# James51332/OceanSimulation

Measured on AMD Instinct MI355X. Metric: height-field points/sec (N² iFFT) at 1/2/4/8 MI355X; % HBM roofline, higher is better.
Workload: dtype f32

## Files before the change

include/oceanfft.h:

```cpp
#ifndef OCEANFFT_H
#define OCEANFFT_H

#include <stddef.h>
#include <stdint.h>

#ifdef __cplusplus
extern "C" {
#endif

#define OCEAN_OK 0
#define OCEAN_ERR_INVALID 1
#define OCEAN_ERR_HIP 2
#define OCEAN_ERR_NO_DEVICE 3
#define OCEAN_ERR_OOM 4

#define OCEAN_MAX_CASCADES 64

typedef struct ocean_settings
{
  int32_t seed[2];
  float U_10;
  float theta_0;
  float F;
  float g;
// ... 44 lines not shown
int ocean_generator_set_frame_overlap(ocean_generator* gen, int enable);
int ocean_generator_frame_bytes(const ocean_generator* gen, double per_point[2]);

int ocean_generator_create_slab(ocean_generator** out, ocean_fft* fft, int rank, int ranks);
size_t ocean_generator_exchange_bytes(const ocean_generator* gen);
int ocean_generator_slab_columns(ocean_generator* gen, float timestep, int update_spectrum, float* send);
int ocean_generator_slab_rows(ocean_generator* gen, const float* recv);
int ocean_generator_slab_info(const ocean_generator* gen, int* rank, int* ranks, int* row0, int* rows);
int ocean_slab_layout(size_t texture_size, int rank, int ranks, int half, int64_t out[6]);

#define OCEAN_COMM_ID_BYTES 128
typedef struct ocean_comm ocean_comm;
int ocean_comm_unique_id(unsigned char id[OCEAN_COMM_ID_BYTES]);
int ocean_comm_create(ocean_comm** out, const unsigned char id[OCEAN_COMM_ID_BYTES], int nranks, int rank);
int ocean_comm_wrap(ocean_comm** out, void* nccl_comm, int nranks, int rank);
int ocean_comm_destroy(ocean_comm* comm);
int ocean_comm_all_to_all(ocean_comm* comm, const void* send, void* recv, size_t bytes, void* hip_stream);
int ocean_generator_slab_frame(ocean_generator* gen, ocean_comm* comm, float timestep, int update_spectrum);
int ocean_generator_slab_frame_pipelined(ocean_generator* gen, ocean_comm* comm, float timestep, int update_spectrum);
int ocean_generator_slab_flush(ocean_generator* gen);

#define OCEAN_ERR_TIMEOUT 5
#define OCEAN_PEER_HANDLE_BYTES 256
typedef struct ocean_peers ocean_peers;
int ocean_peers_create(ocean_peers** out, ocean_generator* gen);
int ocean_peers_destroy(ocean_peers* peers);
int ocean_peers_handle(const ocean_peers* peers, unsigned char handle[OCEAN_PEER_HANDLE_BYTES]);
int ocean_peers_connect(ocean_peers* peers, const unsigned char* handles);
int ocean_peers_connect_local(ocean_peers* const* all, int ranks);
int ocean_peers_set_timeout(ocean_peers* peers, int ms);
int ocean_peers_set_put_cus(ocean_peers* peers, int cus);
int ocean_peers_set_streams(ocean_peers* peers, void* column_stream, void* put_stream, void* row_stream);
int ocean_peers_set_row_cus(ocean_peers* peers, int cus);
int ocean_peers_set_put_cu_mask(ocean_peers* peers, int cus_per_xcd);
int ocean_generator_slab_frame_put(ocean_generator* gen, ocean_peers* peers, float timestep, int update_spectrum);
int ocean_generator_slab_frame_put_pipelined(ocean_generator* gen, ocean_peers* peers, float timestep,
                                             int update_spectrum);
int ocean_peers_flush(ocean_peers* peers);
int ocean_generator_slab_put_columns(ocean_generator* gen, ocean_peers* peers, float timestep, int update_spectrum);
int ocean_generator_slab_put_rows(ocean_generator* gen, ocean_peers* peers);
int ocean_peers_synchronize(ocean_peers* peers);

int ocean_peers_debug_slot(const ocean_peers* peers, int slot, void** ptr, size_t* bytes);

int ocean_frame_plan(size_t texture_size, int cascades, int32_t out[8]);

int ocean_generator_set_profiling(ocean_generator* gen, int enable);
int ocean_generator_kernel_times(ocean_generator* gen, double ms_total[3], int64_t launches[3]);
int ocean_generator_kernel_times4(ocean_generator* gen, double ms_total[4], int64_t launches[4]);

int ocean_debug_hash(const uint32_t* xy, int count, uint32_t* raw, float* uv, void* hip_stream);
int ocean_debug_copy(void* dst, const void* src, size_t bytes, int workgroups, void* hip_stream);
int ocean_debug_fft_work_limit(ocean_fft* fft, size_t bytes);

int ocean_surface_sample(ocean_generator* const* gens, const int* cascades, int count, const float* xz,
                         int64_t points, float* out);
int ocean_surface_sample_plane(ocean_generator* const* gens, const int* cascades, int count, const float camera[5],
                               int res, float* out);
int ocean_surface_query(ocean_generator* const* gens, const int* cascades, int count, const float* xz,
                        int64_t points, int iterations, float tolerance, float* out);

int ocean_generator_mip_levels(const ocean_generator* gen);
int ocean_generator_build_mips(ocean_generator* gen);
float* ocean_generator_height_mip(ocean_generator* gen, int cascade, int level);
float* ocean_generator_displacement_mip(ocean_generator* gen, int cascade, int level);
float* ocean_generator_jacobian_mip(ocean_generator* gen, int cascade, int level);
int ocean_surface_sample_lod(ocean_generator* const* gens, const int* cascades, int count, const float* xzf,
                             int64_t points, float* out);
int ocean_surface_sample_plane_lod(ocean_generator* const* gens, const int* cascades, int count,
                                   const float camera[5], int res, float* out);

int ocean_generator_calculate_rates(ocean_generator* gen);
float* ocean_generator_height_rate_map(ocean_generator* gen, int cascade);
float* ocean_generator_displacement_rate_map(ocean_generator* gen, int cascade);
int ocean_surface_velocity(ocean_generator* const* gens, const int* cascades, int count, const float* xz,
                           int64_t points, float* out);

int ocean_generator_set_depth_layers(ocean_generator* gen, const float* depths, int layers);
int ocean_generator_depth_layers(const ocean_generator* gen, float out[8]);
int ocean_generator_calculate_kinematics(ocean_generator* gen);
float* ocean_generator_kinematics_map(ocean_generator* gen, int cascade, int layer, int image);
int ocean_water_kinematics(ocean_generator* const* gens, const int* cascades, int count, const float* xyz,
                           int64_t points, int iterations, float tolerance, float* out);

int ocean_generator_build_bounds(ocean_generator* gen);
int ocean_generator_bounds(ocean_generator* gen, int cascade, float out[18]);
const float* ocean_generator_bounds_device(ocean_generator* gen);
int ocean_surface_raycast(ocean_generator* const* gens, const int* cascades, int count, const float* rays,
                          int64_t n_rays, float step, int max_steps, int refine, int iterations, float tolerance,
                          float slope, float pad, float* out);

typedef struct ocean_camera
{
  float position[3];
  float right[3], up[3], forward[3];
  float tan_half_fov_y, near_plane, far_plane;
  float lod_scale;
} ocean_camera;
typedef struct ocean_shading
{
  float wave_color[3], scatter_color[3], sky_color[3], light_color[3], light_direction[3];
  float sun_view_angle, sun_falloff_angle, fog_begin, fog_density;
} ocean_shading;
typedef struct ocean_march
{
  float step;
// ... 115 lines not shown
```

oceansimulation_amd/capi.py:

```python
from __future__ import annotations

import ctypes
import os

_HERE = os.path.dirname(os.path.abspath(__file__))
LIB_PATH = os.path.join(_HERE, "liboceanfft.so")

OCEAN_OK = 0
OCEAN_ERR_INVALID = 1
OCEAN_ERR_HIP = 2
OCEAN_ERR_NO_DEVICE = 3
OCEAN_ERR_OOM = 4
OCEAN_ERR_TIMEOUT = 5
OCEAN_MAX_CASCADES = 64
OCEAN_COMM_ID_BYTES = 128
OCEAN_PEER_HANDLE_BYTES = 256


class OceanSettings(ctypes.Structure):

    _fields_ = [
        ("seed", ctypes.c_int32 * 2),
        ("U_10", ctypes.c_float),
        ("theta_0", ctypes.c_float),
# ... 121 lines not shown
        ("foam_hi", ctypes.c_float),
        ("foam_opacity", ctypes.c_float),
        ("spray_color", ctypes.c_float * 3),
        ("spray_radius", ctypes.c_float),
        ("spray_max_half", ctypes.c_int32),
        ("spray_opacity", ctypes.c_float),
    ]


assert ctypes.sizeof(OceanCameraLayers) == 48

_vp = ctypes.c_void_p
_i = ctypes.c_int
_f = ctypes.c_float
_sz = ctypes.c_size_t
_fp = ctypes.POINTER(ctypes.c_float)
_sp = ctypes.POINTER(OceanSettings)
_fsp = ctypes.POINTER(OceanFoamSettings)

SIGNATURES = {
    "ocean_last_error": (ctypes.c_char_p, []),
    "ocean_version": (ctypes.c_char_p, []),
    "ocean_default_settings": (None, [_sp]),
    "ocean_device_count": (_i, []),
    "ocean_fft_create": (_i, [ctypes.POINTER(_vp), _sz, _vp]),
    "ocean_fft_destroy": (_i, [_vp]),
    "ocean_fft_texture_resolution": (_sz, [_vp]),
    "ocean_fft_encode_ifft": (_i, [_vp, _vp]),
    "ocean_fft_encode_ifft_batch": (_i, [_vp, _vp, _i]),
    "ocean_fft_synchronize": (_i, [_vp]),
    "ocean_fft_device_cus": (_i, [_vp]),
    "ocean_fft_set_cu_budget": (_i, [_vp, _i]),
    "ocean_generator_create": (_i, [ctypes.POINTER(_vp), _vp, _i]),
    "ocean_generator_destroy": (_i, [_vp]),
    "ocean_generator_cascades": (_i, [_vp]),
    "ocean_generator_settings": (_sp, [_vp, _i]),
    "ocean_generator_calculate": (_i, [_vp, _f, _i]),
    "ocean_generator_generate_spectrum": (_i, [_vp]),
    "ocean_generator_height_map": (_vp, [_vp, _i]),
    "ocean_generator_displacement_map": (_vp, [_vp, _i]),
    "ocean_generator_jacobian_map": (_vp, [_vp, _i]),
    "ocean_generator_initial_spectrum": (_vp, [_vp, _i]),
    "ocean_generator_spectrum_block": (_i, [_vp]),
    "ocean_generator_create_slab": (_i, [ctypes.POINTER(_vp), _vp, _i, _i]),
    "ocean_generator_exchange_bytes": (_sz, [_vp]),
    "ocean_generator_slab_columns": (_i, [_vp, _f, _i, _vp]),
    "ocean_generator_slab_rows": (_i, [_vp, _vp]),
    "ocean_generator_slab_info": (_i, [_vp, ctypes.POINTER(_i), ctypes.POINTER(_i), ctypes.POINTER(_i), ctypes.POINTER(_i)]),
    "ocean_generator_set_profiling": (_i, [_vp, _i]),
    "ocean_generator_kernel_times": (_i, [_vp, ctypes.POINTER(ctypes.c_double), ctypes.POINTER(ctypes.c_int64)]),
    "ocean_debug_hash": (_i, [_vp, _i, _vp, _vp, _vp]),
    "ocean_debug_copy": (_i, [_vp, _vp, _sz, _i, _vp]),
    "ocean_debug_fft_work_limit": (_i, [_vp, _sz]),
    "ocean_surface_sample": (_i, [_vp, _vp, _i, _vp, ctypes.c_int64, _vp]),
    "ocean_surface_sample_plane": (_i, [_vp, _vp, _i, _vp, _i, _vp]),
    "ocean_surface_query": (_i, [_vp, _vp, _i, _vp, ctypes.c_int64, _i, ctypes.c_float, _vp]),
    "ocean_generator_mip_levels": (_i, [_vp]),
    "ocean_generator_build_mips": (_i, [_vp]),
    "ocean_generator_height_mip": (_vp, [_vp, _i, _i]),
    "ocean_generator_displacement_mip": (_vp, [_vp, _i, _i]),
    "ocean_generator_jacobian_mip": (_vp, [_vp, _i, _i]),
    "ocean_surface_sample_lod": (_i, [_vp, _vp, _i, _vp, ctypes.c_int64, _vp]),
    "ocean_surface_sample_plane_lod": (_i, [_vp, _vp, _i, _vp, _i, _vp]),
    "ocean_generator_calculate_rates": (_i, [_vp]),
    "ocean_generator_height_rate_map": (_vp, [_vp, _i]),
    "ocean_generator_displacement_rate_map": (_vp, [_vp, _i]),
    "ocean_surface_velocity": (_i, [_vp, _vp, _i, _vp, ctypes.c_int64, _vp]),
    "ocean_generator_set_depth_layers": (_i, [_vp, _fp, _i]),
    "ocean_generator_depth_layers": (_i, [_vp, _fp]),
    "ocean_generator_calculate_kinematics": (_i, [_vp]),
    "ocean_generator_kinematics_map": (_vp, [_vp, _i, _i, _i]),
    "ocean_water_kinematics": (_i, [_vp, _vp, _i, _vp, ctypes.c_int64, _i, ctypes.c_float, _vp]),
    "ocean_generator_build_bounds": (_i, [_vp]),
    "ocean_generator_bounds": (_i, [_vp, _i, _fp]),
    "ocean_generator_bounds_device": (_vp, [_vp]),
    "ocean_surface_raycast": (_i, [_vp, _vp, _i, _vp, ctypes.c_int64, _f, _i, _i, _i, _f, _f, _f, _vp]),
    "ocean_default_camera": (None, [ctypes.POINTER(OceanCamera)]),
    "ocean_default_shading": (None, [ctypes.POINTER(OceanShading)]),
    "ocean_default_march": (None, [ctypes.POINTER(OceanMarch)]),
    "ocean_camera_rays": (_i, [ctypes.POINTER(OceanCamera), _i, _i, _vp, _vp]),
    "ocean_camera_render": (_i, [_vp, _vp, _i, ctypes.POINTER(OceanCamera), ctypes.POINTER(OceanShading),
                                 ctypes.POINTER(OceanMarch), _i, _i, _vp, _vp, _vp]),
    "ocean_default_camera_layers": (None, [ctypes.POINTER(OceanCameraLayers)]),
    "ocean_camera_layers_scratch_bytes": (_sz, [_i, _i]),
    "ocean_camera_render_layers": (_i, [_vp, _vp, _i, ctypes.POINTER(OceanCamera), ctypes.POINTER(OceanShading),
                                        ctypes.POINTER(OceanMarch), ctypes.POINTER(OceanCameraLayers), _i, _i, _vp, _vp,
                                        ctypes.c_int64, _vp, _vp, _vp, _vp, _vp]),
    "ocean_default_foam_settings": (None, [_fsp]),
    "ocean_generator_foam_settings": (_fsp, [_vp, _i]),
    "ocean_generator_advance_foam": (_i, [_vp, _f]),
    "ocean_generator_reset_foam": (_i, [_vp]),
    "ocean_generator_foam_map": (_vp, [_vp, _i]),
    "ocean_generator_foam_counts": (_i, [_vp, _i, ctypes.POINTER(ctypes.c_int64)]),
    "ocean_generator_foam_counts_device": (_vp, [_vp]),
    "ocean_surface_sample_foam": (_i, [_vp, _vp, _i, _vp, ctypes.c_int64, _vp]),
    "ocean_surface_sample_plane_foam": (_i, [_vp, _vp, _i, _vp, _i, _vp]),
    "ocean_default_foam_deposit_settings": (None, [ctypes.POINTER(OceanFoamDepositSettings)]),
    "ocean_foam_deposit": (_i, [_vp, _vp, _i, ctypes.POINTER(OceanFoamDepositSettings), _vp, _vp, ctypes.c_int64]),
    "ocean_foam_deposit_counts": (_i, [_vp, ctypes.POINTER(ctypes.c_int64)]),
    "ocean_foam_deposit_counts_device": (_vp, [_vp]),
    "ocean_debug_foam_deposit_merge": (_i, [_i]),
    "ocean_hulls_create":(_i, [ctypes.POINTER(_vp), _vp, _vp, ctypes.c_int64, _vp, _i]),
    "ocean_hulls_destroy": (_i, [_vp]),
    "ocean_hulls_bodies": (_i, [_vp]),
    "ocean_hulls_instance_points": (ctypes.c_int64, [_vp]),
    "ocean_debug_hulls_packing": (_i, [_i]),
# ... 82 lines not shown
```

oceansimulation_amd/csrc/device/fft.h:

```cpp
#pragma once

#include <hip/hip_runtime.h>

#include <cstdint>

#include "device/memory.h"

namespace oceanfft
{

__device__ __forceinline__ float2 operator+(float2 a, float2 b) { return make_float2(a.x + b.x, a.y + b.y); }
__device__ __forceinline__ float2 operator-(float2 a, float2 b) { return make_float2(a.x - b.x, a.y - b.y); }
__device__ __forceinline__ float4 operator+(float4 a, float4 b)
{
  return make_float4(a.x + b.x, a.y + b.y, a.z + b.z, a.w + b.w);
}
__device__ __forceinline__ float4 operator-(float4 a, float4 b)
{
  return make_float4(a.x - b.x, a.y - b.y, a.z - b.z, a.w - b.w);
}
__device__ __forceinline__ float2 mul_i(float2 a) { return make_float2(-a.y, a.x); }
__device__ __forceinline__ float4 mul_i(float4 a) { return make_float4(-a.y, a.x, -a.w, a.z); }
__device__ __forceinline__ float2 mul_mi(float2 a) { return make_float2(a.y, -a.x); }
__device__ __forceinline__ float4 mul_mi(float4 a) { return make_float4(a.y, -a.x, a.w, -a.z); }
// ... 275 lines not shown
#pragma unroll
    for (int u = 0; u < U; u++)
    {
      V w[R0];
#pragma unroll
      for (int t = 0; t < R0; t++)
        w[t] = v[u + t * U];
      if constexpr (R0 == 2)
        idft2(w[0], w[1]);
      else if constexpr (R0 == 4)
        idft4(w[0], w[1], w[2], w[3]);
      else
        idft8(w);
#pragma unroll
      for (int t = 0; t < R0; t++)
        v[u + t * U] = w[t];
    }
    exchange<LOGN, CI, SPLIT, WAVE>(v, reg, i2, reg2, lds, [&](int q) {
      int u = q % U, t = q / U;
      return pad16((i + u * T) * R0 + t);
    });
  }

  int p = R0;
#pragma unroll
  for (int s = 1; s < S::NSTAGE; s++)
  {
    const int k = i2 & (p - 1);
    const int stride = N / (16 * p);
    apply_stage_twiddles<LOGN>(v, k * stride, tw);
    idft16(v);
    if (s + 1 < S::NSTAGE)
    {
      const int j = (i2 / p) * 16 * p + k;
      const int pp = p;
      if (pp >= 16)
      {
        const int base = pad16(j), st = pp + pp / 16;
        exchange<LOGN, CI, SPLIT, WAVE>(v, reg2, i2, reg2, lds, [&](int t) { return base + t * st; });
      }
      else
        exchange<LOGN, CI, SPLIT, WAVE>(v, reg2, i2, reg2, lds, [&](int t) { return pad16(j + t * pp); });
    }
    p *= 16;
  }
}

template <int LOGN, int CI, bool SPLIT, typename V>
__device__ __forceinline__ void fft_run(V* v, int i, int reg, void* lds, const float2* __restrict__ tw)
{
  fft_run<LOGN, CI, SPLIT>(v, i, reg, i, reg, lds, tw);
}

template <int LOGN, int CI>
__device__ __forceinline__ void exchange_x2(CPair* va, CPair* vb, int reg, void* lds_raw, int ia, int ib, int base_a,
                                            int base_b, int st)
{
  using S = FftShape<LOGN>;
  float2* lds = reinterpret_cast<float2*>(lds_raw);
#pragma unroll
  for (int half = 0; half < 2; half++)
  {
#pragma unroll
    for (int t = 0; t < 16; t++)
    {
      lds[lds_slot<CI, S::PADDED>(reg, base_a + t * st)] = half_of(va[t], half);
      lds[lds_slot<CI, S::PADDED>(reg, base_b + t * st)] = half_of(vb[t], half);
    }
    XSYNC();
#pragma unroll
    for (int m = 0; m < 16; m++)
    {
      set_half(va[m], half, lds[lds_slot<CI, S::PADDED>(reg, read_pidx<LOGN>(ia, m))]);
      set_half(vb[m], half, lds[lds_slot<CI, S::PADDED>(reg, read_pidx<LOGN>(ib, m))]);
    }
    XSYNC();
  }
}

template <int LOGN, int CI>
__device__ __forceinline__ void fft_run_x2(CPair* va, CPair* vb, int ia, int reg, void* lds, const float2* __restrict__ tw)
{
  using S = FftShape<LOGN>;
  constexpr int N = S::N, T = S::T;
  static_assert(S::R0 == 16 && CI > 0, "radix-16 stages, column layout");
  const int ib = ia + T / 2;
  idft16(va);
  idft16(vb);
  exchange_x2<LOGN, CI>(va, vb, reg, lds, ia, ib, 17 * ia, 17 * ib, 1);
  int p = 16;
#pragma unroll
  for (int s = 1; s < S::NSTAGE; s++)
  {
    const int stride = N / (16 * p);
    apply_stage_twiddles<LOGN>(va, (ia & (p - 1)) * stride, tw);
    apply_stage_twiddles<LOGN>(vb, (ib & (p - 1)) * stride, tw);
    idft16(va);
    idft16(vb);
    if (s + 1 < S::NSTAGE)
    {
      const int ja = (ia / p) * 16 * p + (ia & (p - 1)), jb = (ib / p) * 16 * p + (ib & (p - 1));
      exchange_x2<LOGN, CI>(va, vb, reg, lds, ia, ib, pad16(ja), pad16(jb), p + p / 16);
    }
    p *= 16;
  }
}
// ... 12 lines not shown
```

oceansimulation_amd/csrc/device/k_half_cols.h:

```cpp
#pragma once

#include <hip/hip_runtime.h>

#include <cstdint>

#include "ocean_internal.h"
#include "launch_common.h"
#include "device/evolve.h"
#include "device/fft.h"
#include "device/grid.h"
#include "device/memory.h"
#include "device/spectrum.h"

namespace oceanfft
{


template <int LOGN>
struct HalfCfg
{
  static constexpr int N = 1 << LOGN;
  static constexpr int B = ColFirstCfg<LOGN>::B;
  static constexpr int STRIPS = N / (2 * B) + 1;
  static constexpr bool SUPPORTED = B == 4 && ColFirstCfg<LOGN>::SPW == 1;
  static constexpr bool SLAB_SUPPORTED = ColFirstCfg<LOGN>::SPW == 1;
};

constexpr int kHalfRG = 2, kHalfRGC = 4;
constexpr int kHalfRG2 = 4, kHalfRGC2 = 8;
constexpr int kHalfHL = 1, kHalfHK = 4, kHalfHKSeed = 2;
template <int LOGN, int RG, int FB = 4>
__device__ __forceinline__ int half_group_offset(int y, int strip, int b = 0)
{
  constexpr int N = HalfCfg<LOGN>::N, FS = HalfCfg<LOGN>::STRIPS * HalfCfg<LOGN>::B / FB;
  return RG == 1 ? (strip * N + y) * FB + b : (((y / RG) * FS + strip) * RG + (y % RG)) * FB + b;
}


template <int LOGN_, bool SEED_>
struct ColsWhole
{
  static constexpr int LOGN = LOGN_, LA = SEED_ ? 0 : kStream;
  static constexpr bool SLAB = false, SEED = SEED_, PUT = false, NYQ = true;
  static constexpr int RG = kHalfRG, RGC = kHalfRGC, FB = 4;
  static constexpr int CPI = ColFirstCfg<LOGN_>::B, HB = ColFirstCfg<LOGN_>::B;
  static constexpr int HL = kHalfHL, HK = SEED_ ? kHalfHKSeed : LOGN_ == 12 ? kHalfHK : 2;
};

template <int LOGN_, bool SEED_, int HB_>
struct ColsHalfStrip
{
  static constexpr int LOGN = LOGN_, LA = SEED_ ? 0 : kStream;
  static constexpr bool SLAB = false, SEED = SEED_, PUT = false, NYQ = true;
  static constexpr int RG = kHalfRG2, RGC = kHalfRGC2, FB = 2;
  static constexpr int CPI = 2, HB = HB_;
  static constexpr int HL = kHalfHL, HK = SEED_ ? kHalfHKSeed : LOGN_ == 12 ? kHalfHK : 2;
};

template <int LOGN_, bool PUT_>
struct ColsSlab
{
  static constexpr int LOGN = LOGN_, LA = kStream;
  static constexpr bool SLAB = true, SEED = false, PUT = PUT_, NYQ = false;
  static constexpr int RG = 1, RGC = 1, FB = 4;
  static constexpr int CPI = ColFirstCfg<LOGN_>::B, HB = ColFirstCfg<LOGN_>::B;
  static constexpr int HL = kHalfHL, HK = LOGN_ == 13 ? 1 : kHalfHK - 1;
};

template <typename Sh>
struct ColsLaunch
{
  using S = FftShape<Sh::LOGN>;
  static constexpr int WG = S::T * Sh::CPI;
  static constexpr int LDS = ((S::TW_ENTRIES * 8 + 15) / 16) * 16 + Sh::CPI * S::PADDED * 8 + Sh::HL * WG * 16;
  static constexpr int items(int cascades, int nstrips) { return cascades * nstrips * (ColFirstCfg<Sh::LOGN>::B / Sh::CPI); }
  static constexpr int max_grid(int hs_blocks) { return Sh::SLAB ? hs_blocks : hs_blocks * (1024 / WG); }
};

template <typename Sh>
__global__ __launch_bounds__(ColsLaunch<Sh>::WG, Sh::CPI < ColFirstCfg<Sh::LOGN>::B ? 4 : 1) void k_cols_half(
    FrameParams fp, const float4* __restrict__ h0, float4* __restrict__ gab, float4* __restrict__ gde,
    float2* __restrict__ gc, const float2* __restrict__ tw_glob, float2* __restrict__ hs, HalfSlab hsl,
    unsigned char* __restrict__ send, int h0_full, const SpectrumConsts* __restrict__ seed)
{
  constexpr int LOGN = Sh::LOGN, LA = Sh::LA, RG = Sh::RG, RGC = Sh::RGC, CPI = Sh::CPI, HL = Sh::HL, HK = Sh::HK,
                FB = Sh::FB, HB = Sh::HB;
  constexpr bool SLAB = Sh::SLAB, SEED = Sh::SEED, PUT = Sh::PUT, NYQ = Sh::NYQ;
  using S = FftShape<LOGN>;
  using K = ColFirstCfg<LOGN>;
  using HC = HalfCfg<LOGN>;
  constexpr int N = S::N, T = S::T, B = K::B, STRIPS = HC::STRIPS, WG = T * CPI, HALVES = B / CPI;
  static_assert(SLAB ? HC::SLAB_SUPPORTED : HC::SUPPORTED, "half-spectrum path: one strip per item (B = 4 unless SLAB)");
  static_assert(CPI * HALVES == B && HALVES <= 2 && (HALVES == 1 || !SLAB), "whole or half strips");
  static_assert(HL >= 0 && HK >= 0 && HL + HK <= 8, "H pairs outside the scratch");
  static_assert(FB == 4 || (FB == CPI && HALVES == 2 && !SLAB && RG > 1 && RGC > 1), "FB: half-strip fields");
  static_assert(!PUT || SLAB, "PUT: the strip-dealt slab stores");
  static_assert(HB == B || (HB == CPI && HALVES == 2 && !SLAB), "HB: half strips over 2-column h0 strips");
  static_assert(!NYQ || !SLAB, "NYQ: whole grids (send is the spec output)");
  constexpr int XB = CPI * S::PADDED * 8;
  extern __shared__ __attribute__((aligned(16))) unsigned char smem[];
  float2* tw = reinterpret_cast<float2*>(smem);
  void* xch = smem + ((S::TW_ENTRIES * 8 + 15) / 16) * 16;
  float4* hlds = reinterpret_cast<float4*>(static_cast<unsigned char*>(xch) + XB);
  load_twiddles<LOGN>(tw, tw_glob);

  const int nstrips = SLAB ? hsl.nstrips : STRIPS;
  const int total = fp.cascades * nstrips * HALVES;
  const float dim = (float)N;
  for (int item = HALVES > 1 ? xcd_pair_slot(blockIdx.x, gridDim.x) : (int)blockIdx.x; item < total; item += gridDim.x)
  {
    const int hh = HALVES > 1 ? item % HALVES : 0, si = HALVES > 1 ? item / HALVES : item;
    const int c = si / nstrips, s = si - c * nstrips;
    const int sg = SLAB ? hsl.strip0 + s : s;
    if (HALVES > 1 && sg == STRIPS - 1 && hh != 0)
      continue;
    const int b = opaque((int)threadIdx.x) % CPI + hh * CPI;
    const int xb = sg == STRIPS - 1 ? 0 : N / (2 * B) + sg;
    const CascadeFrame f = fp.c[c];
    const float4* src = HB != B                  ? h0 + ((size_t)c * (N / HB) + xb * (B / HB) + hh) * N * HB
                        : (!SLAB || h0_full) ? h0 + ((size_t)c * (N / B) + xb) * N * B
                                             : h0 + ((size_t)c * nstrips + s) * N * B;
    const int fs = FB == 4 ? s : 2 * s + hh;
    const size_t gbase = RG == 1 ? ((size_t)c * STRIPS + s) * N * B
                                 : (size_t)c * STRIPS * N * B + half_group_offset<LOGN, RG, FB>(0, fs);
    const size_t cgbase = RGC == 1 ? ((size_t)c * STRIPS + s) * N * B
                                   : (size_t)c * STRIPS * N * B + half_group_offset<LOGN, RGC, FB>(0, fs);
    const int bf = FB == 4 ? b : b - hh * CPI;
    const int x = xb * B + b;
    float4 hk[HK > 0 ? HK : 1];
    auto run_round = [&](int round) __attribute__((always_inline)) {
      const int i = (opaque((int)threadIdx.x) / CPI) % T;
      const int voff = (i * B + b) * 16;
      CPair v[16];
      auto pack = [&](int m, float2 H, const KVec& q) __attribute__((always_inline)) {
        if (round == 0)
          v[m] = CPair{f2v{H.x, q.kz * H.x}, f2v{H.y, q.kz * H.y}};
        else if (round == 1)
        {
          const float e = q.kz * q.dirz;
          v[m] = CPair{f2v{q.dirz * H.x, e * H.x}, f2v{q.dirz * H.y, e * H.y}};
        }
        else
          v[m] = CPair{f2v{q.inv * H.x, 0.0f}, f2v{q.inv * H.y, 0.0f}};
      };
      if (SEED && round == 0)
      {
        float2* hsb = hs + (size_t)blockIdx.x * 16 * WG;
        const int hoff = opaque((int)threadIdx.x) * 8;
        const SpectrumConsts q = seed[c];
#pragma unroll 1
        for (int m = 0; m < 16; m++)
        {
          const int y = i + ((m + 8) & 15) * T;
          const float2 H = evolve(seed_texel(q, x, y, dim), make_kvec(x, y, dim, f.dk).k, f);
          if ((m >> 1) < HL)
            reinterpret_cast<float2*>(hlds)[((m >> 1) * WG + threadIdx.x) * 2 + (m & 1)] = H;
          else
            st2s<0>(hsb, hoff * 2 + (m & 1) * 8, (m >> 1) * WG * 16, H);
        }
        __threadfence_block();
#pragma unroll
        for (int m = 0; m < 16; m += 2)
        {
          const int y = i + ((m + 8) & 15) * T, p = m >> 1;
          const float4 pp = p < HL ? hlds[p * WG + threadIdx.x] : ld4s<kStream>(hsb, hoff * 2, p * WG * 16);
          if (p >= HL && p < HL + HK)
            hk[p < HL + HK && p >= HL ? p - HL : 0] = pp;
          pack(m, make_float2(pp.x, pp.y), make_kvec(x, y, dim, f.dk));
          pack(m + 1, make_float2(pp.z, pp.w), make_kvec(x, y + T, dim, f.dk));
        }
      }
      else if (round == 0)
      {
        float2* hsb = hs + (size_t)blockIdx.x * 16 * WG;
        const int hoff = opaque((int)threadIdx.x) * 8;
        float4 a[16];
        float2 hprev = make_float2(0.0f, 0.0f);
        const int loff = HB == B ? voff : (i * HB + (b - hh * CPI)) * 16;
#pragma unroll
        for (int m = 0; m < 16; m++)
          a[m] = ld4s<LA>(src, loff, ((m + 8) & 15) * T * HB * 16);
#pragma unroll
        for (int m = 0; m < 16; m++)
        {
          const int y = i + ((m + 8) & 15) * T;
          const KVec q = make_kvec(x, y, dim, f.dk);
          const float2 H = evolve(a[m], q.k, f);
          const int p = m >> 1;
          if ((m & 1) && p < HL)
            hlds[p * WG + threadIdx.x] = make_float4(hprev.x, hprev.y, H.x, H.y);
          else if ((m & 1) && p < HL + HK)
            hk[p - HL] = make_float4(hprev.x, hprev.y, H.x, H.y);
          else if (m & 1)
            st4s<0>(hsb, hoff * 2, p * WG * 16, make_float4(hprev.x, hprev.y, H.x, H.y));
          else
            hprev = H;
          pack(m, H, q);
        }
      }
      else
      {
        const float2* hsb = hs + (size_t)blockIdx.x * 16 * WG;
        const int hoff = opaque((int)threadIdx.x) * 8;
#pragma unroll
        for (int m = 0; m < 16; m += 2)
        {
          const int y = i + ((m + 8) & 15) * T, pi = m >> 1;
          const float4 p = pi < HL        ? hlds[pi * WG + threadIdx.x]
                           : pi < HL + HK ? hk[pi < HL + HK ? pi - HL : 0]
                                          : ld4s<kStream>(hsb, hoff * 2, pi * WG * 16);
          pack(m, make_float2(p.x, p.y), make_kvec(x, y, dim, f.dk));
          pack(m + 1, make_float2(p.z, p.w), make_kvec(x, y + T, dim, f.dk));
        }
      }
      const int reg = HALVES > 1 ? opaque((int)threadIdx.x) % CPI : b;
      fft_run<LOGN, CPI, true>(v, i, reg, xch, tw);
      const int vo = (i * B + b) * 16;
#pragma unroll
      for (int m = 0; m < 16; m++)
      {
        if constexpr (SLAB)
        {
          const size_t part = (size_t)fp.cascades * hsl.S * hsl.w * B;
          const int q = (m * T) / hsl.w, yl0 = (m * T) % hsl.w;
          const size_t el = (((size_t)c * hsl.S + s) * hsl.w + yl0) * B;
          unsigned char* blk =
              PUT ? reinterpret_cast<unsigned char*>(sopaque((size_t)reinterpret_cast<const uint64_t*>(send)[q]))
                  : send + sopaque((size_t)q * (part * 40 + (size_t)fp.cascades * 2 * N * 16));
          if (round == 0)
            st4<kStream>(blk + el * 16, vo, pair_raw(v[m]));
          else if (round == 1)
            st4<kStream>(blk + part * 16 + el * 16, vo, pair_raw(v[m]));
          else
            st2<kStream>(blk + part * 32 + el * 8, (i * B + b) * 8, make_float2(v[m].re.x, v[m].im.x));
        }
        else if constexpr (RG == 1 && RGC == 1)
        {
          if (round == 0)
            st4s<kStream>(gab + gbase, vo, m * T * B * 16, pair_raw(v[m]));
          else if (round == 1)
            st4s<kStream>(gde + gbase, vo, m * T * B * 16, pair_raw(v[m]));
          else
            st2s<kStream>(gc + gbase, (i * B + b) * 8, m * T * B * 8, make_float2(v[m].re.x, v[m].im.x));
        }
        else if (round == 0)
          st4s<kStream>(gab + gbase, half_group_offset<LOGN, RG, FB>(i, 0, bf) * 16, half_group_offset<LOGN, RG, FB>(m * T, 0) * 16,
                        pair_raw(v[m]));
        else if (round == 1)
          st4s<kStream>(gde + gbase, half_group_offset<LOGN, RG, FB>(i, 0, bf) * 16, half_group_offset<LOGN, RG, FB>(m * T, 0) * 16,
                        pair_raw(v[m]));
        else
          st2s<kStream>(gc + cgbase, half_group_offset<LOGN, RGC, FB>(i, 0, bf) * 8, half_group_offset<LOGN, RGC, FB>(m * T, 0) * 8,
                        make_float2(v[m].re.x, v[m].im.x));
      }
    };
#pragma unroll
    for (int round = 0; round < 3; round++)
      run_round(round);
  }
  if constexpr (NYQ)
    if ((HALVES > 1 ? xcd_pair_slot(blockIdx.x, gridDim.x) : (int)blockIdx.x) == (int)gridDim.x - 1)
      for (int idx = threadIdx.x; idx < fp.cascades * N; idx += WG)
        half_nyquist_texel(fp, N, HB, h0, reinterpret_cast<float4*>(send), nullptr, 1, 0, seed, nullptr, 0, idx);
}

template <typename Sh>
hipError_t launch_cols_half(const FrameParams& fp, int nstrips, const float4* h0, float4* gab, float4* gde, float2* gc,
                            const float2* tw, float2* hs, int hs_blocks, const HalfSlab& hsl, unsigned char* send,
                            int h0_full, const SpectrumConsts* seed, hipStream_t stream, int cus)
{
  using G = ColsLaunch<Sh>;
  auto kern = k_cols_half<Sh>;
  int grid = persistent_grid(kern, G::WG, G::LDS, G::items(fp.cascades, nstrips), cus);
  if (grid > G::max_grid(hs_blocks))
    grid = G::max_grid(hs_blocks);
  if (grid < 1)
    return hipErrorInvalidValue;
  hipLaunchKernelGGL(kern, dim3(grid), dim3(G::WG), G::LDS, stream, fp, h0, gab, gde, gc, tw, hs, hsl, send, h0_full, seed);
  return hipGetLastError();
}

}
```

oceansimulation_amd/csrc/device/memory.h:

```cpp
#pragma once

#include <hip/hip_runtime.h>

#include <cstdint>


namespace oceanfft
{

typedef float f4v __attribute__((ext_vector_type(4)));

__device__ __forceinline__ __amdgpu_buffer_rsrc_t srd(const void* base, int num_bytes)
{
  return __builtin_amdgcn_make_buffer_rsrc(const_cast<void*>(base), 0, num_bytes, 0x00020000);
}

constexpr int kAllBytes = 0x7FFFFFFF;

template <int AUX = 0>
__device__ __forceinline__ float4 ld4(const void* base, int voff_bytes, int num_bytes = kAllBytes)
{
  f4v r = __builtin_amdgcn_raw_buffer_load_b128(srd(base, num_bytes), voff_bytes, 0, AUX);
  return make_float4(r.x, r.y, r.z, r.w);
}
// ... 22 lines not shown
}

template <int AUX = 0>
__device__ __forceinline__ void st1(void* base, int voff_bytes, float v)
{
  __builtin_amdgcn_raw_buffer_store_b32(__float_as_uint(v), srd(base, kAllBytes), voff_bytes, 0, AUX);
}

#if defined(OCEAN_SOFFSET_PIECES)
#define OCEAN_PIECE(voff, soff) (voff), (soff)
#else
#define OCEAN_PIECE(voff, soff) (voff) + (soff), 0
#endif
template <int AUX = 0>
__device__ __forceinline__ float4 ld4s(const void* base, int voff_bytes, int soff_bytes)
{
  f4v r = __builtin_amdgcn_raw_buffer_load_b128(srd(base, kAllBytes), OCEAN_PIECE(voff_bytes, soff_bytes), AUX);
  return make_float4(r.x, r.y, r.z, r.w);
}

template <int AUX = 0>
__device__ __forceinline__ void st4s(void* base, int voff_bytes, int soff_bytes, float4 v)
{
  f4v r = {v.x, v.y, v.z, v.w};
  __builtin_amdgcn_raw_buffer_store_b128(r, srd(base, kAllBytes), OCEAN_PIECE(voff_bytes, soff_bytes), AUX);
}

template <int AUX = 0>
__device__ __forceinline__ float2 ld2s(const void* base, int voff_bytes, int soff_bytes)
{
  u2v r = __builtin_amdgcn_raw_buffer_load_b64(srd(base, kAllBytes), OCEAN_PIECE(voff_bytes, soff_bytes), AUX);
  return make_float2(__uint_as_float(r.x), __uint_as_float(r.y));
}

template <int AUX = 0>
__device__ __forceinline__ void st2s(void* base, int voff_bytes, int soff_bytes, float2 v)
{
  u2v r = {__float_as_uint(v.x), __float_as_uint(v.y)};
  __builtin_amdgcn_raw_buffer_store_b64(r, srd(base, kAllBytes), OCEAN_PIECE(voff_bytes, soff_bytes), AUX);
}

__device__ __forceinline__ int clamp_bytes(int64_t b)
{
  return b > kAllBytes ? kAllBytes : (b < 0 ? 0 : (int)b);
}


__device__ __forceinline__ int opaque(int v)
{
  asm volatile("" : "+v"(v));
  return v;
}

__device__ __forceinline__ size_t sopaque(size_t v)
{
  asm volatile("" : "+s"(v));
  return v;
}

__device__ __forceinline__ int sopaque(int v)
{
  asm volatile("" : "+s"(v));
  return v;
}

}
```

oceansimulation_amd/csrc/launch_half.hip:

```cpp
#include <hip/hip_runtime.h>

#include <cstdint>

#include "oceanfft.h"
#include "ocean_internal.h"
#include "launch_common.h"
#include "device/grid.h"
#include "device/k_half_cols.h"
#include "device/k_half_rows.h"
#include "device/k_rows_hp.h"
#include "device/spectrum.h"

namespace oceanfft
{

bool half_spectrum_supported(int logn) { return logn >= 10 && logn <= 12; }

constexpr bool half_strip_launch(int logn, int cascades) { return (logn == 12 || logn == 11) && cascades <= 2; }

template <int LOGN, typename V>
hipError_t select_half_cols(int cascades, bool seed, int h0_blk, V&& visit)
{
  constexpr int B = ColFirstCfg<LOGN>::B;
  if constexpr (LOGN == 12 || LOGN == 11)
// ... 25 lines not shown

template <int LOGN, typename V>
hipError_t select_half_rows(int cascades, V&& visit)
{
  const bool hs = half_strip_launch(LOGN, cascades);
  if constexpr (LOGN == 12)
    return hs ? visit(RowsHp<2, kHalfRG2, kHalfRGC2, kHalfRGC2, 0, 4>{}) : visit(RowsHp<4, kHalfRG, kHalfRGC, 4, 1, 3>{});
  else if constexpr (LOGN == 11)
    return hs ? visit(RowsHalf<2, kHalfRG2, kHalfRGC2>{}) : visit(RowsHalf<4, kHalfRG, kHalfRGC>{});
  else
    return visit(RowsHalf<4, kHalfRG, kHalfRGC>{});
}

int half_h0_block(int logn, int cascades)
{
  int hb = spectrum_block(logn);
  (void)with_logn(logn, [&](auto L) -> hipError_t {
    constexpr int LOGN = decltype(L)::value;
    if constexpr (HalfCfg<LOGN>::SUPPORTED)
      return select_half_cols<LOGN>(cascades, false, 0, [&](auto sh) {
        hb = decltype(sh)::HB;
        return hipSuccess;
      });
    else
      return hipSuccess;
  });
  return hb;
}

size_t half_field_texels(int logn)
{
  const size_t n = (size_t)1 << logn;
  return (n / 8 + 1) * n * 4;
}

size_t half_hs_bytes(int logn, int blocks)
{
  return half_slab_supported(logn) ? (size_t)blocks * 16 * 1024 * sizeof(float2) : 0;
}

hipError_t launch_half_columns(int logn, const FrameParams& fp, const float4* h0, float4* gab, float4* gcd, float2* ge,
                               float4* spec, const float2* tw, hipStream_t stream, int cus, float2* hs, int hs_blocks,
                               const void* seed_consts, int h0_blk)
{
  if (!hs)
    return hipErrorInvalidValue;
  const SpectrumConsts* seed = static_cast<const SpectrumConsts*>(seed_consts);
  return with_logn(logn, [&](auto L) -> hipError_t {
    constexpr int LOGN = decltype(L)::value;
    if constexpr (!HalfCfg<LOGN>::SUPPORTED)
      return hipErrorInvalidValue;
    else
      return select_half_cols<LOGN>(fp.cascades, seed != nullptr, h0_blk > 0 ? h0_blk : ColFirstCfg<LOGN>::B, [&](auto sh) {
        return launch_cols_half<decltype(sh)>(fp, HalfCfg<LOGN>::STRIPS, h0, gab, gcd, ge, tw, hs, hs_blocks, HalfSlab{},
                                              reinterpret_cast<unsigned char*>(spec), 1, seed, stream, cus);
      });
  });
}

hipError_t launch_half_rows(int logn, const FrameParams& fp, const float4* gab, const float4* gcd, const float2* ge,
                            const float4* rcorr, float4* maps, float* jac, const FoamParams& foam, const float2* tw,
                            hipStream_t stream, int cus)
{
  return with_logn(logn, [&](auto L) -> hipError_t {
    constexpr int LOGN = decltype(L)::value;
    if constexpr (!HalfCfg<LOGN>::SUPPORTED)
      return hipErrorInvalidValue;
    else
      return select_half_rows<LOGN>(fp.cascades, [&](auto sh) {
        using R = decltype(sh);
        using S = FftShape<LOGN>;
        if constexpr (R::HP)
        {
          auto kern = k_rows_hp<R::RG, R::RGC, false, R::FB, R::GRP, R::EARLY, R::MINB>;
          const int grid = persistent_grid(kern, 256, HpCfg::LDS, fp.cascades * S::N, cus);
          hipLaunchKernelGGL(kern, dim3(grid), dim3(256), HpCfg::LDS, stream, fp, gab, gcd, ge, rcorr, maps, jac, foam, tw, 0,
                             RowSrc{});
        }
        else
        {
          auto kern = k_rows_half<LOGN, 0, false, R::RG, R::RGC, R::FB>;
          const int lds = ((S::TW_ENTRIES * 8 + 15) / 16) * 16 + lds_row_slots<LOGN>(2) * 8;
          const int grid = persistent_grid(kern, S::T * 2, lds, fp.cascades * (S::N / 2), cus);
          hipLaunchKernelGGL(kern, dim3(grid), dim3(S::T * 2), lds, stream, fp, gab, gcd, ge, rcorr, maps, jac, foam, tw, S::N,
                             RowSrc{});
        }
        return hipGetLastError();
      });
  });
}

}

extern "C" int ocean_frame_plan(size_t texture_size, int cascades, int32_t out[8])
{
  using namespace oceanfft;
  int logn = 0;
  while (logn < 15 && ((size_t)1 << logn) < texture_size)
    logn++;
  if (!out || ((size_t)1 << logn) != texture_size || !half_spectrum_supported(logn) || cascades < 1 ||
      cascades > kMaxCascades)
    return OCEAN_ERR_INVALID;
  const hipError_t e = with_logn(logn, [&](auto L) -> hipError_t {
    constexpr int LOGN = decltype(L)::value;
    if constexpr (!HalfCfg<LOGN>::SUPPORTED)
      return hipErrorInvalidValue;
    else
// ... 20 lines not shown
```

oceansimulation_amd/csrc/ocean_capi.cpp:

```cpp
#include "oceanfft.h"

#include <hip/hip_runtime.h>

#include <algorithm>
#include <cmath>
#include <cstdio>
#include <cstring>
#include <string>
#include <vector>

#include "ocean_capi_internal.h"
#include "ocean_internal.h"

static_assert(sizeof(ocean_settings) == sizeof(OceanSettings), "settings layout");

namespace
{
int log2_exact(size_t n)
{
  int l = 0;
  while (((size_t)1 << l) < n)
    l++;
  return ((size_t)1 << l) == n ? l : -1;
}
// ... 224 lines not shown
{
  if (!fft)
    return fail(OCEAN_ERR_INVALID, "ocean_fft_synchronize: null plan");
  HIP_TRY(hipStreamSynchronize(fft->stream), "hipStreamSynchronize");
  return OCEAN_OK;
}

}

namespace
{
hipEvent_t take_event(ocean_generator* g)
{
  if (!g->pool.empty())
  {
    hipEvent_t e = g->pool.back();
    g->pool.pop_back();
    return e;
  }
  hipEvent_t e = nullptr;
  (void)hipEventCreate(&e);
  return e;
}

template <typename F>
hipError_t timed(ocean_generator* g, int kind, F&& launch, hipStream_t stream = nullptr)
{
  if (!g->profiling)
    return launch();
  if (!stream)
    stream = g->fft->stream;
  EventPair p{kind, take_event(g), take_event(g)};
  hipError_t e = hipEventRecord(p.a, stream);
  if (e != hipSuccess)
    return e;
  e = launch();
  if (e != hipSuccess)
    return e;
  e = hipEventRecord(p.b, stream);
  g->pending.push_back(p);
  return e;
}

hipError_t half_fields(ocean_generator* g, int slot)
{
  const size_t t = half_field_texels(g->fft->logn) * g->cascades;
  HalfFields& f = g->fields[slot];
  hipError_t e = alloc_if_null(f.gab, t * sizeof(float4));
  e = alloc_if_null(f.gde, t * sizeof(float4), e);
  e = alloc_if_null(f.gc, t * sizeof(float2), e);
  return alloc_if_null(f.spec, (size_t)g->cascades * 2 * g->fft->n * sizeof(float4), e);
}

hipError_t half_buffers(ocean_generator* g)
{
  return alloc_if_null(g->hs, half_hs_bytes(g->fft->logn, g->fft->device_cus), half_fields(g, 0));
}

HalfSlab half_slab_geom(int logn, int rank, int ranks)
{
  const int strips = half_strips(logn);
  HalfSlab h{};
  h.S = (strips + ranks - 1) / ranks;
  h.strip0 = rank * h.S;
  h.nstrips = std::max(0, std::min(h.S, strips - h.strip0));
  h.w = (1 << logn) / ranks;
  return h;
}

int h0_block(const ocean_generator* g)
{
  switch (frame_path(g))
  {
    case FramePath::FourStep:
      return gen4_h0_block();
    case FramePath::HalfBlocked:
      return half_h0_block(g->fft->logn, g->cascades);
    default:
      return spectrum_block(g->fft->logn);
  }
}

size_t h0_texels(const ocean_generator* g)
{
  const size_t full = (size_t)g->fft->n * g->geom.w;
  if (g->ranks == 1)
    return full;
  const size_t strips = (size_t)g->hsl.nstrips * spectrum_block(g->fft->logn) * g->fft->n;
  size_t t = std::max(full, strips);
  if (gen4_supported(g->fft->logn))
    t = std::max(t, g->g4.h0_cstride);
  return t;
}

hipError_t full_buffers(ocean_generator* g)
{
  const size_t slab = (size_t)g->fft->n * g->geom.w * g->cascades;
  hipError_t e = alloc_if_null(g->inter, slab * 2 * sizeof(float4));
  return rows_need_transpose(g->fft->logn) ? alloc_if_null(g->scratch, slab * 2 * sizeof(float4), e) : e;
}

hipError_t path_buffers(ocean_generator* g)
{
  switch (frame_path(g))
  {
    case FramePath::Full:
// ... 825 lines not shown
```

Baseline: 61.37 billion.

## Carry the last column strip into spare FFT lanes of the third round for N=1024

For the 1024 whole-grid column kernel, the last strip is no longer given its own work items. Blocks with s==0 or s==1 compute that strip's extra fields in the unused .y lanes of the round-2 FFT and store them separately. The Nyquist texel pass is also spread across all blocks instead of running on the last block only. This aims to remove a tail of poorly occupied work and improve load balance, at the cost of extra registers, h0 loads, and opaque scheduling barriers in the round-2 path.

```diff
diff --git a/include/oceanfft.h b/include/oceanfft.h
--- a/include/oceanfft.h
+++ b/include/oceanfft.h
@@ -120,6 +120,7 @@
 int ocean_debug_hash(const uint32_t* xy, int count, uint32_t* raw, float* uv, void* hip_stream);
 int ocean_debug_copy(void* dst, const void* src, size_t bytes, int workgroups, void* hip_stream);
 int ocean_debug_fft_work_limit(ocean_fft* fft, size_t bytes);
+int ocean_debug_fill_half_fields(ocean_generator* gen, int byte);
 
 int ocean_surface_sample(ocean_generator* const* gens, const int* cascades, int count, const float* xz,
                          int64_t points, float* out);
diff --git a/oceansimulation_amd/capi.py b/oceansimulation_amd/capi.py
--- a/oceansimulation_amd/capi.py
+++ b/oceansimulation_amd/capi.py
@@ -197,6 +197,7 @@
     "ocean_debug_hash": (_i, [_vp, _i, _vp, _vp, _vp]),
     "ocean_debug_copy": (_i, [_vp, _vp, _sz, _i, _vp]),
     "ocean_debug_fft_work_limit": (_i, [_vp, _sz]),
+    "ocean_debug_fill_half_fields": (_i, [_vp, _i]),
     "ocean_surface_sample": (_i, [_vp, _vp, _i, _vp, ctypes.c_int64, _vp]),
     "ocean_surface_sample_plane": (_i, [_vp, _vp, _i, _vp, _i, _vp]),
     "ocean_surface_query": (_i, [_vp, _vp, _i, _vp, ctypes.c_int64, _i, ctypes.c_float, _vp]),
diff --git a/oceansimulation_amd/csrc/device/fft.h b/oceansimulation_amd/csrc/device/fft.h
--- a/oceansimulation_amd/csrc/device/fft.h
+++ b/oceansimulation_amd/csrc/device/fft.h
@@ -351,6 +351,79 @@
   fft_run<LOGN, CI, SPLIT>(v, i, reg, i, reg, lds, tw);
 }
 
+template <int LOGN, typename V>
+__device__ __forceinline__ void fft_stage0(V* v)
+{
+  using S = FftShape<LOGN>;
+  constexpr int R0 = S::R0;
+  if constexpr (R0 == 16)
+    idft16(v);
+  else
+  {
+    constexpr int U = 16 / R0;
+#pragma unroll
+    for (int u = 0; u < U; u++)
+    {
+      V w[R0];
+#pragma unroll
+      for (int t = 0; t < R0; t++)
+        w[t] = v[u + t * U];
+      if constexpr (R0 == 2)
+        idft2(w[0], w[1]);
+      else if constexpr (R0 == 4)
+        idft4(w[0], w[1], w[2], w[3]);
+      else
+        idft8(w);
+#pragma unroll
+      for (int t = 0; t < R0; t++)
+        v[u + t * U] = w[t];
+    }
+  }
+}
+
+template <int LOGN, int CI, bool SPLIT, typename V>
+__device__ __forceinline__ void fft_after_stage0(V* v, int i, int reg, void* lds, const float2* __restrict__ tw)
+{
+  using S = FftShape<LOGN>;
+  constexpr int N = S::N, T = S::T, R0 = S::R0;
+  static_assert(S::NSTAGE > 1, "a transform with an exchange");
+  if constexpr (R0 == 16)
+  {
+    const int base = 17 * i;
+    exchange<LOGN, CI, SPLIT>(v, reg, i, reg, lds, [&](int t) { return base + t; });
+  }
+  else
+  {
+    constexpr int U = 16 / R0;
+    exchange<LOGN, CI, SPLIT>(v, reg, i, reg, lds, [&](int q) {
+      int u = q % U, t = q / U;
+      return pad16((i + u * T) * R0 + t);
+    });
+  }
+  int p = R0;
+#pragma unroll
+  for (int s = 1; s < S::NSTAGE; s++)
+  {
+    const int k = i & (p - 1);
+    const int stride = N / (16 * p);
+    apply_stage_twiddles<LOGN>(v, k * stride, tw);
+    idft16(v);
+    if (s + 1 < S::NSTAGE)
+    {
+      const int j = (i / p) * 16 * p + k;
+      const int pp = p;
+      if (pp >= 16)
+      {
+        const int base = pad16(j), st = pp + pp / 16;
+        exchange<LOGN, CI, SPLIT>(v, reg, i, reg, lds, [&](int t) { return base + t * st; });
+      }
+      else
+        exchange<LOGN, CI, SPLIT>(v, reg, i, reg, lds, [&](int t) { return pad16(j + t * pp); });
+    }
+    p *= 16;
+  }
+}
+
 template <int LOGN, int CI>
 __device__ __forceinline__ void exchange_x2(CPair* va, CPair* vb, int reg, void* lds_raw, int ia, int ib, int base_a,
                                             int base_b, int st)
diff --git a/oceansimulation_amd/csrc/device/k_half_cols.h b/oceansimulation_amd/csrc/device/k_half_cols.h
--- a/oceansimulation_amd/csrc/device/k_half_cols.h
+++ b/oceansimulation_amd/csrc/device/k_half_cols.h
@@ -3,6 +3,7 @@
 #include <hip/hip_runtime.h>
 
 #include <cstdint>
+#include <type_traits>
 
 #include "ocean_internal.h"
 #include "launch_common.h"
@@ -41,7 +42,7 @@
 struct ColsWhole
 {
   static constexpr int LOGN = LOGN_, LA = SEED_ ? 0 : kStream;
-  static constexpr bool SLAB = false, SEED = SEED_, PUT = false, NYQ = true;
+  static constexpr bool SLAB = false, SEED = SEED_, PUT = false, NYQ = true, CARRY = !SEED_ && LOGN_ == 10;
   static constexpr int RG = kHalfRG, RGC = kHalfRGC, FB = 4;
   static constexpr int CPI = ColFirstCfg<LOGN_>::B, HB = ColFirstCfg<LOGN_>::B;
   static constexpr int HL = kHalfHL, HK = SEED_ ? kHalfHKSeed : LOGN_ == 12 ? kHalfHK : 2;
@@ -51,7 +52,7 @@
 struct ColsHalfStrip
 {
   static constexpr int LOGN = LOGN_, LA = SEED_ ? 0 : kStream;
-  static constexpr bool SLAB = false, SEED = SEED_, PUT = false, NYQ = true;
+  static constexpr bool SLAB = false, SEED = SEED_, PUT = false, NYQ = true, CARRY = false;
   static constexpr int RG = kHalfRG2, RGC = kHalfRGC2, FB = 2;
   static constexpr int CPI = 2, HB = HB_;
   static constexpr int HL = kHalfHL, HK = SEED_ ? kHalfHKSeed : LOGN_ == 12 ? kHalfHK : 2;
@@ -61,7 +62,7 @@
 struct ColsSlab
 {
   static constexpr int LOGN = LOGN_, LA = kStream;
-  static constexpr bool SLAB = true, SEED = false, PUT = PUT_, NYQ = false;
+  static constexpr bool SLAB = true, SEED = false, PUT = PUT_, NYQ = false, CARRY = false;
   static constexpr int RG = 1, RGC = 1, FB = 4;
   static constexpr int CPI = ColFirstCfg<LOGN_>::B, HB = ColFirstCfg<LOGN_>::B;
   static constexpr int HL = kHalfHL, HK = LOGN_ == 13 ? 1 : kHalfHK - 1;
@@ -73,19 +74,26 @@
   using S = FftShape<Sh::LOGN>;
   static constexpr int WG = S::T * Sh::CPI;
   static constexpr int LDS = ((S::TW_ENTRIES * 8 + 15) / 16) * 16 + Sh::CPI * S::PADDED * 8 + Sh::HL * WG * 16;
+  static constexpr int GRID_STRIPS = HalfCfg<Sh::LOGN>::STRIPS - (Sh::CARRY ? 1 : 0);
   static constexpr int items(int cascades, int nstrips) { return cascades * nstrips * (ColFirstCfg<Sh::LOGN>::B / Sh::CPI); }
   static constexpr int max_grid(int hs_blocks) { return Sh::SLAB ? hs_blocks : hs_blocks * (1024 / WG); }
 };
 
+__device__ __forceinline__ float quad_odd(float v)
+{
+  const int r = __float_as_int(v);
+  return __int_as_float(__builtin_amdgcn_update_dpp(r, r, 0xF5 , 0xF, 0xF, true));
+}
+
 template <typename Sh>
-__global__ __launch_bounds__(ColsLaunch<Sh>::WG, Sh::CPI < ColFirstCfg<Sh::LOGN>::B ? 4 : 1) void k_cols_half(
+__global__ __launch_bounds__(ColsLaunch<Sh>::WG, Sh::CPI < ColFirstCfg<Sh::LOGN>::B || Sh::CARRY ? 4 : 1) void k_cols_half(
     FrameParams fp, const float4* __restrict__ h0, float4* __restrict__ gab, float4* __restrict__ gde,
     float2* __restrict__ gc, const float2* __restrict__ tw_glob, float2* __restrict__ hs, HalfSlab hsl,
     unsigned char* __restrict__ send, int h0_full, const SpectrumConsts* __restrict__ seed)
 {
   constexpr int LOGN = Sh::LOGN, LA = Sh::LA, RG = Sh::RG, RGC = Sh::RGC, CPI = Sh::CPI, HL = Sh::HL, HK = Sh::HK,
                 FB = Sh::FB, HB = Sh::HB;
-  constexpr bool SLAB = Sh::SLAB, SEED = Sh::SEED, PUT = Sh::PUT, NYQ = Sh::NYQ;
+  constexpr bool SLAB = Sh::SLAB, SEED = Sh::SEED, PUT = Sh::PUT, NYQ = Sh::NYQ, CARRY = Sh::CARRY;
   using S = FftShape<LOGN>;
   using K = ColFirstCfg<LOGN>;
   using HC = HalfCfg<LOGN>;
@@ -97,6 +105,8 @@
   static_assert(!PUT || SLAB, "PUT: the strip-dealt slab stores");
   static_assert(HB == B || (HB == CPI && HALVES == 2 && !SLAB), "HB: half strips over 2-column h0 strips");
   static_assert(!NYQ || !SLAB, "NYQ: whole grids (send is the spec output)");
+  static_assert(!CARRY || (!SLAB && !SEED && HALVES == 1 && B == 4 && FB == 4 && HB == B && RG > 1 && RGC > 1),
+                "CARRY: whole strips of whole grids that load h0");
   constexpr int XB = CPI * S::PADDED * 8;
   extern __shared__ __attribute__((aligned(16))) unsigned char smem[];
   float2* tw = reinterpret_cast<float2*>(smem);
@@ -104,7 +114,7 @@
   float4* hlds = reinterpret_cast<float4*>(static_cast<unsigned char*>(xch) + XB);
   load_twiddles<LOGN>(tw, tw_glob);
 
-  const int nstrips = SLAB ? hsl.nstrips : STRIPS;
+  const int nstrips = SLAB ? hsl.nstrips : CARRY ? STRIPS - 1 : STRIPS;
   const int total = fp.cascades * nstrips * HALVES;
   const float dim = (float)N;
   for (int item = HALVES > 1 ? xcd_pair_slot(blockIdx.x, gridDim.x) : (int)blockIdx.x; item < total; item += gridDim.x)
@@ -128,7 +138,8 @@
     const int bf = FB == 4 ? b : b - hh * CPI;
     const int x = xb * B + b;
     float4 hk[HK > 0 ? HK : 1];
-    auto run_round = [&](int round) __attribute__((always_inline)) {
+    auto run_round = [&](int round, auto cy) __attribute__((always_inline)) {
+      constexpr int CY = decltype(cy)::value;
       const int i = (opaque((int)threadIdx.x) / CPI) % T;
       const int voff = (i * B + b) * 16;
       CPair v[16];
@@ -214,7 +225,56 @@
         }
       }
       const int reg = HALVES > 1 ? opaque((int)threadIdx.x) % CPI : b;
-      fft_run<LOGN, CPI, true>(v, i, reg, xch, tw);
+      if constexpr (CY != 0)
+      {
+        fft_stage0<LOGN>(v);
+#pragma unroll
+        for (int m = 0; m < 16; m++)
+          v[m].re.x = fopaque(v[m].re.x), v[m].im.x = fopaque(v[m].im.x);
+        CPair w[16];
+        const int cf = CY == 2 ? 4 : b;
+        const float4* nsrc = h0 + (size_t)c * N * N;
+        const int noff = i * B * 16;
+        constexpr int NG = 4;
+#pragma unroll
+        for (int g = 0; g < 16; g += NG)
+        {
+          float4 a[NG];
+          __builtin_amdgcn_sched_barrier(0);
+#pragma unroll
+          for (int j = 0; j < NG; j++)
+            a[j] = ld4s<LA>(nsrc, noff, ((g + j + 8) & 15) * T * B * 16);
+          const int ig = opaque(i);
+#pragma unroll
+          for (int j = 0; j < NG; j++)
+          {
+            const int m = g + j, y = ig + ((m + 8) & 15) * T;
+            const KVec q = make_kvec(0, y, dim, f.dk);
+            float2 H = evolve(a[j], q.k, f);
+            if constexpr (CY == 2)
+            {
+              H.x = fopaque(H.x), H.y = fopaque(H.y);
+              const float inv = fopaque(q.inv);
+              w[m] = CPair{f2v{inv * H.x, 0.0f}, f2v{inv * H.y, 0.0f}};
+            }
+            else
+            {
+              const float kz = fopaque(q.kz), dirz = fopaque(q.dirz), e = fopaque(kz * dirz);
+              const float fac = cf == 1 ? kz : cf == 2 ? dirz : e;
+              const float wx = fac * H.x, wy = fac * H.y;
+              w[m] = CPair{f2v{fopaque(cf == 0 ? H.x : wx), 0.0f}, f2v{fopaque(cf == 0 ? H.y : wy), 0.0f}};
+            }
+            __builtin_amdgcn_sched_barrier(0);
+          }
+        }
+        fft_stage0<LOGN>(w);
+#pragma unroll
+        for (int m = 0; m < 16; m++)
+          v[m].re.y = w[m].re.x, v[m].im.y = w[m].im.x;
+        fft_after_stage0<LOGN, CPI, true>(v, i, reg, xch, tw);
+      }
+      else
+        fft_run<LOGN, CPI, true>(v, i, reg, xch, tw);
       const int vo = (i * B + b) * 16;
 #pragma unroll
       for (int m = 0; m < 16; m++)
@@ -253,12 +313,53 @@
           st2s<kStream>(gc + cgbase, half_group_offset<LOGN, RGC, FB>(i, 0, bf) * 8, half_group_offset<LOGN, RGC, FB>(m * T, 0) * 8,
                         make_float2(v[m].re.x, v[m].im.x));
       }
+      if constexpr (CY != 0)
+      {
+        const size_t nb = (size_t)c * STRIPS * N * B + half_group_offset<LOGN, RG, FB>(0, STRIPS - 1);
+        const size_t cnb = (size_t)c * STRIPS * N * B + half_group_offset<LOGN, RGC, FB>(0, STRIPS - 1);
+#pragma unroll
+        for (int m = 0; m < 16; m++)
+        {
+          if constexpr (CY == 2)
+          {
+            if (b == 0)
+              st2s<kStream>(gc + cnb, half_group_offset<LOGN, RGC, FB>(i, 0) * 8, half_group_offset<LOGN, RGC, FB>(m * T, 0) * 8,
+                            make_float2(v[m].re.y, v[m].im.y));
+          }
+          else
+          {
+            const float4 t = make_float4(v[m].re.y, quad_odd(v[m].re.y), v[m].im.y, quad_odd(v[m].im.y));
+            const int go = half_group_offset<LOGN, RG, FB>(i, 0) * 16, gs = half_group_offset<LOGN, RG, FB>(m * T, 0) * 16;
+            if (b == 0)
+              st4s<kStream>(gab + nb, go, gs, t);
+            else if (b == 2)
+              st4s<kStream>(gde + nb, go, gs, t);
+          }
+        }
+      }
     };
-#pragma unroll
-    for (int round = 0; round < 3; round++)
-      run_round(round);
+    if constexpr (!CARRY)
+    {
+#pragma unroll
+      for (int round = 0; round < 3; round++)
+        run_round(round, std::integral_constant<int, 0>{});
+    }
+    else
+    {
+      run_round(0, std::integral_constant<int, 0>{});
+      run_round(1, std::integral_constant<int, 0>{});
+      if (s == 0)
+        run_round(2, std::integral_constant<int, 1>{});
+      else if (s == 1)
+        run_round(2, std::integral_constant<int, 2>{});
+      else
+        run_round(2, std::integral_constant<int, 0>{});
+    }
   }
-  if constexpr (NYQ)
+  if constexpr (NYQ && CARRY)
+    for (int idx = blockIdx.x * WG + threadIdx.x; idx < fp.cascades * N; idx += gridDim.x * WG)
+      half_nyquist_texel(fp, N, HB, h0, reinterpret_cast<float4*>(send), nullptr, 1, 0, seed, nullptr, 0, idx);
+  else if constexpr (NYQ)
     if ((HALVES > 1 ? xcd_pair_slot(blockIdx.x, gridDim.x) : (int)blockIdx.x) == (int)gridDim.x - 1)
       for (int idx = threadIdx.x; idx < fp.cascades * N; idx += WG)
         half_nyquist_texel(fp, N, HB, h0, reinterpret_cast<float4*>(send), nullptr, 1, 0, seed, nullptr, 0, idx);
diff --git a/oceansimulation_amd/csrc/device/memory.h b/oceansimulation_amd/csrc/device/memory.h
--- a/oceansimulation_amd/csrc/device/memory.h
+++ b/oceansimulation_amd/csrc/device/memory.h
@@ -98,6 +98,12 @@
   return v;
 }
 
+__device__ __forceinline__ float fopaque(float v)
+{
+  asm volatile("" : "+v"(v));
+  return v;
+}
+
 __device__ __forceinline__ size_t sopaque(size_t v)
 {
   asm volatile("" : "+s"(v));
diff --git a/oceansimulation_amd/csrc/launch_half.hip b/oceansimulation_amd/csrc/launch_half.hip
--- a/oceansimulation_amd/csrc/launch_half.hip
+++ b/oceansimulation_amd/csrc/launch_half.hip
@@ -101,7 +101,7 @@
       return hipErrorInvalidValue;
     else
       return select_half_cols<LOGN>(fp.cascades, seed != nullptr, h0_blk > 0 ? h0_blk : ColFirstCfg<LOGN>::B, [&](auto sh) {
-        return launch_cols_half<decltype(sh)>(fp, HalfCfg<LOGN>::STRIPS, h0, gab, gcd, ge, tw, hs, hs_blocks, HalfSlab{},
+        return launch_cols_half<decltype(sh)>(fp, ColsLaunch<decltype(sh)>::GRID_STRIPS, h0, gab, gcd, ge, tw, hs, hs_blocks, HalfSlab{},
                                               reinterpret_cast<unsigned char*>(spec), 1, seed, stream, cus);
       });
   });
diff --git a/oceansimulation_amd/csrc/ocean_capi.cpp b/oceansimulation_amd/csrc/ocean_capi.cpp
--- a/oceansimulation_amd/csrc/ocean_capi.cpp
+++ b/oceansimulation_amd/csrc/ocean_capi.cpp
@@ -300,6 +300,25 @@
   return alloc_if_null(f.spec, (size_t)g->cascades * 2 * g->fft->n * sizeof(float4), e);
 }
 
+}
+
+int ocean_debug_fill_half_fields(ocean_generator* g, int byte)
+{
+  if (!g || !g->fields[0].gab)
+    return fail(OCEAN_ERR_INVALID, "ocean_debug_fill_half_fields: no generator, or no blocked half-spectrum frame yet");
+  const size_t t = half_field_texels(g->fft->logn) * g->cascades;
+  for (const HalfFields& f : g->fields)
+    if (f.gab && f.gde && f.gc)
+    {
+      HIP_TRY(hipMemsetAsync(f.gab, byte, t * sizeof(float4), g->fft->stream), "hipMemsetAsync");
+      HIP_TRY(hipMemsetAsync(f.gde, byte, t * sizeof(float4), g->fft->stream), "hipMemsetAsync");
+      HIP_TRY(hipMemsetAsync(f.gc, byte, t * sizeof(float2), g->fft->stream), "hipMemsetAsync");
+    }
+  return OCEAN_OK;
+}
+
+namespace
+{
 hipError_t half_buffers(ocean_generator* g)
 {
   return alloc_if_null(g->hs, half_hs_bytes(g->fft->logn, g->fft->device_cus), half_fields(g, 0));
```

After: 61.39 billion (median of 2 runs). No clear change (+0.0%).
